# mbdriscoll/indigo

Measured on AMD Instinct MI355X. Metric: SENSE AHA evals/sec (256^3 x 8-coil non-Cartesian), higher is better.
Workload: dtype complex64 (f32)

## Files before the change

indigo_amd/csrc/ig_common.h:

```cpp
#pragma once

#include <hip/hip_runtime.h>
#include <cstdint>
#include <cstdio>
#include <cstdarg>
#include <string>
#include <type_traits>
#include <vector>

#include "indigo_hip.h"

struct ig_prof_rec {
    const char* name;
    double      bytes;
    hipEvent_t  e0, e1;
};

struct ig_ctx {
    int          device      = 0;
    hipStream_t  stream      = nullptr;
    bool         own_stream  = false;
    int          num_cu      = 256;
    std::string  err;
    double*      d_partials  = nullptr;
    double*      h_result    = nullptr;
    double*      d_scalars   = nullptr;
    void*        d_xpack     = nullptr;
    size_t       xpack_bytes = 0;
    void*        d_epg       = nullptr;
    size_t       epg_bytes   = 0;
    int32_t*     d_worklist  = nullptr;
    size_t       worklist_bytes = 0, partials_bytes = 0, scalars_bytes = 0;
    int          opt_fft_kernels = 0;
    int          opt_fft_zc = 1;
    bool         bricks_attr = false;
    bool         fft3d_attr = false;
    bool         fft_w32_attr = false;
    bool         fft_lds_attr = false;
    bool                     prof_on = false;
    bool                     capturing = false;
    std::vector<ig_prof_rec> prof;
    std::vector<hipEvent_t>  prof_pool;
};

struct ig_prof_scope {
    ig_ctx* ctx; size_t idx; bool on;
    ig_prof_scope(ig_ctx* c, const char* name, double bytes = 0.0) : ctx(c), idx(0), on(c && c->prof_on) {
        if (!on) return;
        ig_prof_rec r; r.name = name; r.bytes = bytes;
        auto get = [&]() { hipEvent_t e = nullptr;
            if (!ctx->prof_pool.empty()) { e = ctx->prof_pool.back(); ctx->prof_pool.pop_back(); }
            else (void)hipEventCreate(&e);
            return e; };
        r.e0 = get(); r.e1 = get();
        (void)hipEventRecord(r.e0, ctx->stream);
        idx = ctx->prof.size();
        ctx->prof.push_back(r);
    }
    ~ig_prof_scope() { if (on) (void)hipEventRecord(ctx->prof[idx].e1, ctx->stream); }
};

struct ig_graph {
    ig_ctx*        ctx  = nullptr;
    hipGraph_t     graph = nullptr;
    hipGraphExec_t exec = nullptr;
};

struct ig_event {
    ig_ctx*    ctx = nullptr;
    hipEvent_t ev  = nullptr;
};

constexpr int IG_MAX_RED_BLOCKS = 2048;
constexpr int IG_NUM_SCALARS = 1024;

std::string& ig_tls_error();

int ig_fail(ig_ctx* ctx, int code, const char* fmt, ...) __attribute__((format(printf, 3, 4)));

#define IG_HIP(ctx, call)                                                              \
    do {                                                                               \
        hipError_t e_ = (call);                                                        \
        if (e_ != hipSuccess)                                                          \
            return ig_fail((ctx), IG_ERR_HIP, "%s failed: %s (%s:%d)", #call,          \
                           hipGetErrorString(e_), __FILE__, __LINE__);                 \
    } while (0)

#define IG_REQUIRE(ctx, cond, ...)                                                     \
    do {                                                                               \
        if (!(cond)) return ig_fail((ctx), IG_ERR_ARG, __VA_ARGS__);                   \
    } while (0)

// ... 117 lines not shown
```

indigo_amd/csrc/ig_context.hip:

```cpp
#include "ig_common.h"
#include <cstring>

std::string& ig_tls_error() {
    static thread_local std::string e;
    return e;
}

int ig_fail(ig_ctx* ctx, int code, const char* fmt, ...) {
    char buf[1024];
    va_list ap;
    va_start(ap, fmt);
    vsnprintf(buf, sizeof(buf), fmt, ap);
    va_end(ap);
    ig_tls_error() = buf;
    if (ctx) ctx->err = buf;
    return code;
}

extern "C" {

int ig_abi_version(void) { return IG_ABI_VERSION; }

int ig_device_count(int* count) {
    if (!count) return ig_fail(nullptr, IG_ERR_ARG, "ig_device_count: count is NULL");
// ... 37 lines not shown
        ctx->own_stream = false;
    } else {
        if ((e = hipStreamCreateWithFlags(&ctx->stream, hipStreamNonBlocking)) != hipSuccess)
            return bail("hipStreamCreateWithFlags", e);
        ctx->own_stream = true;
    }
    ctx->partials_bytes = sizeof(double) * 2 * (IG_MAX_RED_BLOCKS + 1);
    if ((e = hipMalloc((void**)&ctx->d_partials, ctx->partials_bytes)) != hipSuccess)
        return bail("hipMalloc(partials)", e);
    if ((e = hipHostMalloc((void**)&ctx->h_result, sizeof(double) * 2, hipHostMallocDefault)) != hipSuccess)
        return bail("hipHostMalloc(result)", e);
    *out = ctx;
    return IG_OK;
}

int ig_init(int device_id, ig_ctx** out) { return ig_init_common(device_id, false, nullptr, out); }

int ig_init_on_stream(int device_id, void* hip_stream, ig_ctx** out) {
    return ig_init_common(device_id, true, hip_stream, out);
}

void ig_destroy(ig_ctx* ctx) {
    if (!ctx) return;
    (void)hipSetDevice(ctx->device);
    (void)hipStreamSynchronize(ctx->stream);
    for (ig_prof_rec& r : ctx->prof) { (void)hipEventDestroy(r.e0); (void)hipEventDestroy(r.e1); }
    for (hipEvent_t e : ctx->prof_pool) (void)hipEventDestroy(e);
    if (ctx->d_partials) (void)hipFree(ctx->d_partials);
    if (ctx->d_scalars) (void)hipFree(ctx->d_scalars);
    if (ctx->d_worklist) (void)hipFree(ctx->d_worklist);
    if (ctx->d_xpack) (void)hipFree(ctx->d_xpack);
    if (ctx->d_epg) (void)hipFree(ctx->d_epg);
    if (ctx->h_result) (void)hipHostFree(ctx->h_result);
    if (ctx->own_stream && ctx->stream) (void)hipStreamDestroy(ctx->stream);
    delete ctx;
}

const char* ig_last_error(ig_ctx* ctx) {
    if (ctx) return ctx->err.c_str();
    return ig_tls_error().c_str();
}

int ig_sync(ig_ctx* ctx) {
    IG_REQUIRE(ctx, ctx != nullptr, "ig_sync: ctx is NULL");
    if (int rc = ig_set_device(ctx)) return rc;
    IG_HIP(ctx, hipStreamSynchronize(ctx->stream));
    return IG_OK;
}

void* ig_stream(ig_ctx* ctx) { return ctx ? (void*)ctx->stream : nullptr; }

int ig_graph_begin(ig_ctx* ctx) {
    IG_REQUIRE(ctx, ctx != nullptr, "ig_graph_begin: ctx is NULL");
    IG_REQUIRE(ctx, !ctx->capturing, "ig_graph_begin: already recording");
    IG_REQUIRE(ctx, !ctx->prof_on, "ig_graph_begin: profile mode brackets launches with events of its own; switch it off");
    if (int rc = ig_set_device(ctx)) return rc;
    IG_HIP(ctx, hipStreamBeginCapture(ctx->stream, hipStreamCaptureModeThreadLocal));
    ctx->capturing = true;
    return IG_OK;
}

int ig_graph_end(ig_ctx* ctx, ig_graph** out) {
    IG_REQUIRE(ctx, ctx && out, "ig_graph_end: bad arguments");
    IG_REQUIRE(ctx, ctx->capturing, "ig_graph_end: not recording");
    *out = nullptr;
    ctx->capturing = false;
// ... 34 lines not shown
    ig_ctx* ctx = graph->ctx;
    IG_REQUIRE(ctx, !ctx->capturing, "ig_graph_launch: the context is recording");
    if (int rc = ig_set_device(ctx)) return rc;
    IG_HIP(ctx, hipGraphLaunch(graph->exec, ctx->stream));
    return IG_OK;
}

int ig_graph_destroy(ig_graph* graph) {
    if (!graph) return IG_OK;
    if (graph->exec) (void)hipGraphExecDestroy(graph->exec);
    if (graph->graph) (void)hipGraphDestroy(graph->graph);
    delete graph;
    return IG_OK;
}

int ig_device_name(ig_ctx* ctx, char* buf, size_t len) {
    IG_REQUIRE(ctx, ctx && buf && len > 0, "ig_device_name: bad arguments");
    hipDeviceProp_t prop;
    IG_HIP(ctx, hipGetDeviceProperties(&prop, ctx->device));
    snprintf(buf, len, "%s (%s, %d CUs)", prop.name, prop.gcnArchName, prop.multiProcessorCount);
    return IG_OK;
}

int ig_set_option(ig_ctx* ctx, const char* name, int64_t value) {
    IG_REQUIRE(ctx, ctx && name, "ig_set_option: bad arguments");
    if (std::string(name) == "fft.kernels") {
        IG_REQUIRE(ctx, value >= 0 && value <= 2, "ig_set_option: fft.kernels is 0 (all), 1 (no A x B passes) or 2 (generic stages only)");
        ctx->opt_fft_kernels = (int)value;
        return IG_OK;
    }
    if (std::string(name) == "fft.zc_intermediate") {
        IG_REQUIRE(ctx, value == 0 || value == 1, "ig_set_option: fft.zc_intermediate is 0 (the grid's order) or 1 (z-contiguous per kx tile)");
        ctx->opt_fft_zc = (int)value;
        return IG_OK;
    }
    return ig_fail(ctx, IG_ERR_ARG, "ig_set_option: unknown option '%s'", name);
}

int ig_library_bytes(ig_ctx* ctx, size_t* bytes) {
    IG_REQUIRE(ctx, ctx && bytes, "ig_library_bytes: bad arguments");
    *bytes = ctx->xpack_bytes + ctx->epg_bytes + (ctx->d_worklist ? ctx->worklist_bytes : 0) + (ctx->d_partials ? ctx->partials_bytes : 0) +
             (ctx->d_scalars ? ctx->scalars_bytes : 0);
    return IG_OK;
}

int ig_mem_info(ig_ctx* ctx, size_t* free_bytes, size_t* total_bytes) {
    IG_REQUIRE(ctx, ctx && free_bytes && total_bytes, "ig_mem_info: bad arguments");
    if (int rc = ig_set_device(ctx)) return rc;
    IG_HIP(ctx, hipMemGetInfo(free_bytes, total_bytes));
    return IG_OK;
}


int ig_malloc(ig_ctx* ctx, size_t nbytes, void** dptr) {
    IG_REQUIRE(ctx, ctx && dptr, "ig_malloc: bad arguments");
    if (int rc = ig_set_device(ctx)) return rc;
    *dptr = nullptr;
    size_t n = nbytes ? nbytes : 256;
    hipError_t e = hipMalloc(dptr, n);
    if (e == hipErrorOutOfMemory) {
        (void)hipGetLastError();
        return ig_fail(ctx, IG_ERR_NOMEM, "ig_malloc: out of device memory requesting %zu bytes", nbytes);
    }
    if (e != hipSuccess) return ig_fail(ctx, IG_ERR_HIP, "hipMalloc(%zu) failed: %s", nbytes, hipGetErrorString(e));
    return IG_OK;
}
// ... 156 lines not shown
```

indigo_amd/csrc/ig_fft.hip:

```cpp
#include "ig_common.h"
#include "ig_packed.h"
#include "ig_fft_ab.h"
#include "ig_fft_plan.h"
#include "ig_fft_regs.h"

namespace {


template <int R1, int R2, int T, int W, bool AXIS0, int WMODE, bool BOXED, int HALF>
__global__ void __launch_bounds__(W * T, (!AXIS0 && R1 == 32 && (W == 32 || HALF == 1 || HALF == 3)) ? 4 : 1)
k_fft_2stage(PassDesc d, const float2* __restrict__ tw) {
    constexpr int n = R1 * R2, B1 = R2 / T, B2 = R1 / T, NT = W * T;
    constexpr bool NT_LD = true, NT_ST = true;
    constexpr bool HALF_IN = HALF == 1 || HALF == 3, HALF_OUT = HALF == 2 || HALF == 4;
    constexpr int SUMW = WMODE >= 3 ? (1 << (WMODE - 3)) : 0;
    constexpr bool SINV = HALF_OUT;
    const bool inv = (HALF_OUT || HALF_IN) ? false : (d.inverse != 0);
    static_assert(R2 % T == 0 && R1 % T == 0 && T == 16 && B1 == 1, "lane groups of 16, one stage-1 butterfly per thread");
    extern __shared__ float2 lds[];
    float2* __restrict__ tws = lds + (AXIS0 ? 16 * 17 * W : 16 * T * W);
    const int tid = threadIdx.x;
    constexpr int TWN = n / NT;
    constexpr bool TW_LATE = (n % NT == 0) && TWN <= 2;
    float2 tw_mine[TW_LATE ? TWN : 1];
    if (TW_LATE) {
#pragma unroll
        for (int i = 0; i < TWN; ++i) tw_mine[i] = tw[n + tid + i * NT];
    } else for (int k = tid; k < n; k += NT) tws[k] = tw[n + k];

    const int t = AXIS0 ? (tid % T) : (tid / W);
    const int w = AXIS0 ? (tid / T) : (tid % W);
    unsigned tr, k1, k2;
    pass_tile(d, tr, k1, k2);
    const int64_t k0u = (int64_t)tr * ((!AXIS0 && d.cw) ? (d.cw_log2 >= 0 ? W >> d.cw_log2 : W / d.cw) : W);
    int in_lo = d.in_lo, in_hi = d.in_hi, out_lo = d.out_lo, out_hi = d.out_hi;
    short2 k1r = make_short2(0, 0x7fff), trg = make_short2(0, 0x7fff);
    PassRecords rcd{0u, 0u, 0x7fff0000u, 0xffffffffu, false, false, false, true, false};
    if (BOXED && !AXIS0) rcd = pass_records(d, tw, tr, k1, 16, t, true);
    const bool has_k1r = rcd.has_k1r, has_trg = rcd.has_trg, has_zb = rcd.has_zb;
    int64_t o_in = k0u * d.in_s[0], o_out = k0u * d.out_s[0];
    if (BOXED && !AXIS0 && WMODE == 0 && d.zc_log2) {
        const int64_t q = k0u >> d.zc_log2, e = k0u - (q << d.zc_log2);
        if (d.in_zt) o_in = q * d.in_zt + e;
        if (d.out_zt) o_out = q * d.out_zt + e;
    }
    const float2* const b_in = d.in + (o_in + (int64_t)k1 * d.in_s[1] + (int64_t)k2 * d.in_s[2]);
// ... 194 lines not shown
               "ig_fft: axis stride too large for the %s kernel", kernel);
    return IG_OK;
}

bool ig_two_stage_variant(const AxisPlan& ax, const PassDesc& d, bool axis0, int wmode, bool& boxed, int& half) {
    boxed = d.tile_range || !(d.in_lo <= 0 && d.in_hi >= (int)ax.n && d.out_lo <= 0 && d.out_hi >= (int)ax.n);
    const int qn = (int)ax.n / 4;
    half = 0;
    if (boxed) {
        const bool in_full = d.in_lo <= 0 && d.in_hi >= (int)ax.n, out_full = d.out_lo <= 0 && d.out_hi >= (int)ax.n;
        if (d.in_lo == qn && d.in_hi == 3 * qn && !(d.tile_range && d.tile_range_mode == 2))
            half = (out_full && !d.tile_range && !d.tile_bits) ? 3 : 1;
        else if (d.out_lo == qn && d.out_hi == 3 * qn && !(d.tile_range && d.tile_range_mode == 1))
            half = (in_full && !d.tile_range && !d.tile_bits) ? 4 : 2;
        if (wmode == 1 && half != 3) half = 0;
        if (wmode >= 2 && half != 4) half = 0;
        if (((half == 1 || half == 3) && d.inverse) || ((half == 2 || half == 4) && !d.inverse)) half = 0;
    }
    const bool big_stride = (d.in_sj > d.out_sj ? d.in_sj : d.out_sj) * 8 >= (1 << 20);
    const bool w32_generic = half == 0 && (big_stride || d.tile_bits != nullptr);
    const bool w32 = (ax.n == 512 && !axis0 && wmode == 0 && !d.cw && d.ext0 % 32 == 0 &&
        (half == 1 || half == 3 || half == 2 || half == 4 || w32_generic) &&
        (!d.tile_range || d.tile_shift >= 1));
    return d.wide ? d.wide == 2 : w32;
}


typedef void (*Kernel2S)(PassDesc, const float2*);
template <int WM, int HF> struct V2 {};
template <typename... P> struct V2List {};
using V2_BOXED = V2List<V2<0, 0>, V2<0, 1>, V2<0, 2>, V2<0, 3>, V2<0, 4>, V2<1, 0>, V2<1, 3>, V2<2, 0>, V2<2, 4>>;
using V2_SUM = V2List<V2<3, 0>, V2<3, 4>, V2<4, 0>, V2<4, 4>, V2<5, 0>, V2<5, 4>, V2<6, 0>, V2<6, 4>, V2<7, 0>, V2<7, 4>>;
using V2_W32 = V2List<V2<0, 0>, V2<0, 1>, V2<0, 2>, V2<0, 3>, V2<0, 4>>;
template <int R1, int W, bool AXIS0, int... WM, int... HF>
static Kernel2S pick_2stage(V2List<V2<WM, HF>...>, int wm, int half) {
    Kernel2S k = nullptr;
    ((wm == WM && half == HF ? (void)(k = &k_fft_2stage<R1, 16, 16, W, AXIS0, WM, true, HF>) : (void)0), ...);
    return k;
}

int ig_launch_2stage(ig_ctx* ctx, const AxisPlan& ax, const PassDesc& d_in, bool axis0, int wmode) {
    PassDesc d = d_in;
    if (d.ncols == 0) return IG_OK;
    IG_REQUIRE(ctx, !d.tile_bits || d.tile_words == 16 || d.tile_words == 0, "ig_fft: the two-stage kernel reads support bitmaps of 16 words per entry (got %d)", d.tile_words);
    const int64_t cpt = (!axis0 && d.cw) ? ax.W / d.cw : ax.W;
    IG_REQUIRE(ctx, !d.cw || (!axis0 && d.cw <= ax.W && ax.W % d.cw == 0), "ig_fft: bad lane split");
    dim3 grid, block((unsigned)(ax.W * ax.T));
    if (int rc = ig_pass_tiles(ctx, d, cpt, axis0 ? ax.n + 15 : 3 * (ax.n / 16) + 15, wmode != 0, "two-stage", grid)) return rc;
    size_t lds = ax.lds_bytes;
    bool boxed; int half;
    Kernel2S k = nullptr;
    if (ig_two_stage_variant(ax, d, axis0, wmode, boxed, half)) {
        if (d.tile_range) d.tile_shift -= 1;
        grid = pass_grid(d, d.ext0 / 32); block = dim3(512);
        lds = ((size_t)16 * 16 * 32 + 512) * 8;
        if (!ctx->fft_w32_attr) {
            for (int h = 0; h <= 4; ++h)
                IG_HIP(ctx, hipFuncSetAttribute(reinterpret_cast<const void*>(pick_2stage<32, 32, false>(V2_W32{}, 0, h)), hipFuncAttributeMaxDynamicSharedMemorySize, (int)lds));
            ctx->fft_w32_attr = true;
        }
        k = pick_2stage<32, 32, false>(V2_W32{}, 0, half);
    } else {
        IG_REQUIRE(ctx, wmode != 3 || (!axis0 && d.cw >= 1), "ig_fft: the coil-summing pass is a strided pass with a lane split");
        const int wm = wmode == 3 ? 3 + d.cw_log2 : wmode;
        with_flag(ax.n == 512, [&](auto n512) { with_flag(axis0, [&](auto a0) {
            constexpr int R1 = decltype(n512)::value ? 32 : 16;
            constexpr bool A0 = decltype(a0)::value;
            if (!boxed && wm == 0) k = &k_fft_2stage<R1, 16, 16, 16, A0, 0, false, 0>;
            else if (wm < 3) k = pick_2stage<R1, 16, A0>(V2_BOXED{}, wm, half);
            else if constexpr (!A0) k = pick_2stage<R1, 16, false>(V2_SUM{}, wm, half);
        }); });
    }
    IG_REQUIRE(ctx, k, "ig_fft: no two-stage kernel for weight mode %d", wmode);
    hipLaunchKernelGGL(k, grid, block, lds, ctx->stream, d, ax.d_tw);
    IG_LAUNCH_CHECK(ctx, "k_fft_2stage");
    return IG_OK;
}
```

indigo_amd/csrc/ig_fft_plan.h:

```cpp
#pragma once
#include "ig_common.h"
#include "ig_fft_ab.h"
#include <memory>
#include <string>
#include <vector>

namespace {

constexpr int MAX_STAGES = 16;
constexpr int E = 8;
constexpr int LDS_NMAX = 4096;
constexpr size_t LDS_BUDGET = 150 * 1024;

struct Radices { int r[MAX_STAGES]; };

}

struct Chirp;
struct AxisPlan {
    int64_t n = 1, inner = 1, outer = 1;
    int kind = 2;
    std::shared_ptr<Chirp> chirp;
    int nstages = 0;
    int ab_A = 0, ab_B = 0;
// ... 14 lines not shown
    float2* d_in_s[2] = {nullptr, nullptr};
    float2* d_hat_out_s[2] = {nullptr, nullptr};
    AxisPlan sub;
    bool fused = false;
    ~Chirp() {
        for (int d = 0; d < 2; ++d) { if (d_b[d]) (void)hipFree(d_b[d]); if (d_bhat[d]) (void)hipFree(d_bhat[d]); if (d_bout[d]) (void)hipFree(d_bout[d]);
                                      if (d_hat_out[d]) (void)hipFree(d_hat_out[d]);
                                      if (d_in_s[d]) (void)hipFree(d_in_s[d]); if (d_hat_out_s[d]) (void)hipFree(d_hat_out_s[d]); }
        if (sub.d_tw) (void)hipFree(sub.d_tw);
    }
};

struct ig_fft {
    ig_ctx* ctx = nullptr;
    bool is_chirp_sub = false;
    int rank = 0;
    int64_t dims[3] = {1, 1, 1};
    int64_t batch = 1;
    int64_t total = 0;
    AxisPlan axis[3];
    size_t workspace_bytes = 0;
    std::string desc;
    bool two_launch = false;
    size_t inplace_workspace_bytes = 0;
    bool padded = false;
    bool has_ab_axis = false;
    bool has_chirp_axis = false;
    int zw_in = 16, zw_out = 16;
    int layout = 0;
    int support_tile = 16;
    int64_t box_lo[3] = {0, 0, 0}, box_dims[3] = {1, 1, 1};
};

int ig_launch_2stage(ig_ctx* ctx, const AxisPlan& ax, const PassDesc& d, bool axis0, int wmode);
bool ig_two_stage_variant(const AxisPlan& ax, const PassDesc& d, bool axis0, int wmode, bool& boxed, int& half);
int ig_pass_tiles(ig_ctx* ctx, PassDesc& d, int64_t cpt, int64_t reach, bool weights, const char* kernel, dim3& grid);

int ig_launch_fft3d_a(ig_ctx* ctx, const float2* in, float2* out, const float2* tw, int64_t batch, int inverse);
int ig_launch_fft3d_b(ig_ctx* ctx, const float2* in, float2* out, const float2* tw, int64_t batch, int inverse);
int ig_launch_fft_lds(ig_ctx* ctx, const AxisPlan& ax, const float2* in, float2* out, int inverse);
int ig_launch_fft_generic_stage(ig_ctx* ctx, unsigned blocks, const float2* in, float2* out, const float2* tw, int64_t n, int64_t inner,
                                int64_t total, int R, int64_t Ns, int inverse);
int ig_launch_chirp_pre(ig_ctx* ctx, unsigned blocks, const float2* x, float2* W, const float2* b, int64_t n, int64_t m, int64_t inner, int64_t total_m);
int ig_launch_chirp_mul(ig_ctx* ctx, unsigned blocks, float2* W, const float2* bhat, int64_t m, int64_t inner, int64_t total_m);
int ig_launch_chirp_post(ig_ctx* ctx, unsigned blocks, const float2* W, float2* y, const float2* bout, int64_t n, int64_t m, int64_t inner, int64_t total_n);
```

indigo_amd/csrc/ig_fft_plan.hip:

```cpp
#include "ig_common.h"
#include "ig_fft_ab.h"
#include "ig_fft_ab_list.h"
#include "ig_fft_zc.h"
#include "ig_fft_plan.h"
#include <algorithm>
#include <array>
#include <cmath>
#include <complex>
#include <functional>

namespace {

bool factor_lds(int64_t n, Radices& rad, int& nstages) {
    nstages = 0;
    int64_t m = n;
    auto push = [&](int r) { rad.r[nstages++] = r; };
    while (m % 8 == 0 && nstages < MAX_STAGES) { push(8); m /= 8; }
    while (m % 4 == 0 && nstages < MAX_STAGES) { push(4); m /= 4; }
    while (m % 2 == 0 && nstages < MAX_STAGES) { push(2); m /= 2; }
    for (int p : {3, 5, 7})
        while (m % p == 0 && nstages < MAX_STAGES) { push(p); m /= p; }
    return m == 1;
}

void factor_generic(int64_t n, std::vector<int64_t>& out) {
    out.clear();
    int64_t m = n;
    while (m % 8 == 0) { out.push_back(8); m /= 8; }
    while (m % 4 == 0) { out.push_back(4); m /= 4; }
    while (m % 2 == 0) { out.push_back(2); m /= 2; }
    for (int64_t p = 3; p * p <= m; p += 2)
        while (m % p == 0) { out.push_back(p); m /= p; }
    if (m > 1) out.push_back(m);
}

int64_t largest_prime_factor(int64_t n) {
// ... 266 lines not shown
        }
        upload(hat_out_s[dir], 2 * (size_t)m);
    }
    if (err != hipSuccess) {
        for (int d = 0; d < 2; ++d) { if (in_s[d]) (void)hipFree(in_s[d]); if (hat_out_s[d]) (void)hipFree(hat_out_s[d]); }
        return ig_fail(ctx, IG_ERR_HIP, "ig_fft_set_axis_shift: the tables of a shift by %lld points could not be uploaded: %s", (long long)c, hipGetErrorString(err));
    }
    for (int d = 0; d < 2; ++d) { ch.d_in_s[d] = in_s[d]; ch.d_hat_out_s[d] = hat_out_s[d]; }
    ch.shift = c;
    return IG_OK;
}

int launch_chirp_desc(ig_ctx* ctx, const AxisPlan& ax, const PassDesc& d_in) {
    const Chirp& ch = *ax.chirp;
    IG_REQUIRE(ctx, ch.fused, "ig_fft: this chirp-z axis has no one-launch route");
    IG_REQUIRE(ctx, !d_in.cw && (!d_in.tile_bits || d_in.tile_words == ch.sub.ab_B), "ig_fft: a chirp-z pass takes no lane split, and support bitmaps of B = %d words per entry", ch.sub.ab_B);
    IG_REQUIRE(ctx, d_in.in_lo >= 0 && d_in.in_hi <= ax.n && d_in.out_lo >= 0 && d_in.out_hi <= ax.n, "ig_fft: chirp-z boxes must lie inside the axis");
    PassDesc d = d_in;
    if (d.ncols == 0) return IG_OK;
    const int dir = d.inverse ? 1 : 0;
    d.w = ch.d_b[dir]; d.w2 = ch.d_hat_out[dir]; d.chirp_out = 0;
    if (ch.shift) { d.w = ch.d_in_s[dir]; d.w2 = ch.d_hat_out_s[dir]; d.chirp_out = 1; }
    dim3 grid;
    if (int rc = ig_pass_tiles(ctx, d, anyfft::AB_W, ch.sub.ab_B - 1, false, "chirp-z", grid)) return rc;
    const dim3 block((unsigned)(anyfft::AB_W * ch.sub.ab_B));
    const int r = launch_part(ABZ_PARTS, ctx->stream, ch.m, grid, block, d, ch.sub.d_tw);
    if (r == 2) return ig_fail(ctx, IG_ERR_UNSUPPORTED, "ig_fft: device %d refused the LDS the chirp-z kernel over %lld points needs", ctx->device, (long long)ch.m);
    if (!r)
        return ig_fail(ctx, IG_ERR_UNSUPPORTED, "ig_fft: no chirp-z kernel for m = %lld", (long long)ch.m);
    IG_LAUNCH_CHECK(ctx, "k_fft_chirp");
    return IG_OK;
}

int launch_pass(ig_ctx* ctx, const AxisPlan& ax, const PassDesc& d, bool axis0, int wmode) {
    if (ax.kind == 3) return ig_launch_2stage(ctx, ax, d, axis0, wmode);
    if (ax.kind == 5) {
        IG_REQUIRE(ctx, !axis0 && wmode == 0, "ig_fft: a chirp-z axis takes unweighted strided passes only");
        return launch_chirp_desc(ctx, ax, d);
    }
    IG_REQUIRE(ctx, ax.kind == 4 && !axis0, "ig_fft: a zero-padded pass on an axis without a two-stage kernel");
    return launch_ab_desc(ctx, ax, d, wmode);
}

}

extern "C" {

int ig_fft_plan(ig_ctx* ctx, int rank, const int64_t* dims, int64_t batch, ig_fft** plan, size_t* workspace_bytes) {
    IG_REQUIRE(ctx, ctx && dims && plan, "ig_fft_plan: bad arguments");
    IG_REQUIRE(ctx, rank >= 1 && rank <= 3, "ig_fft_plan: rank %d not in 1..3", rank);
    IG_REQUIRE(ctx, batch >= 1, "ig_fft_plan: batch must be >= 1");
    *plan = nullptr;
    if (int rc = ig_set_device(ctx)) return rc;
    ig_fft* p = new ig_fft();
    p->ctx = ctx; p->rank = rank; p->batch = batch;
    p->total = batch;
    for (int a = 0; a < rank; ++a) {
        if (dims[a] < 1) { delete p; return ig_fail(ctx, IG_ERR_ARG, "ig_fft_plan: dims[%d] = %lld", a, (long long)dims[a]); }
        p->dims[a] = dims[a];
        p->total *= dims[a];
    }
    bool need_ws = false;
    for (int a = 0; a < rank; ++a) {
        int rc = plan_axis(ctx, p, a);
        if (rc != IG_OK) { ig_fft_destroy(p); return rc; }
        if (p->axis[a].kind == 1) need_ws = true;
    }
    p->workspace_bytes = need_ws ? (size_t)p->total * 8 : 0;
// ... 288 lines not shown
    if (g.snt) {
        d.tile_range = support; d.tile_range_mode = inverse ? 2 : 1; d.tile_range_k1 = g.snt; d.tile_shift = g.tile_shift;
    }
    if (support) {
        d.tile_bits = reinterpret_cast<const uint32_t*>(support + g.bits) + (inverse ? 0 : g.bits_out);
        d.tile_words = inverse ? g.zw_in : g.zw_out;
        if (inverse) d.k1_range = support + g.hull_y;
    }
    return d;
}

static bool zc_route(const ig_fft* p, const PaddedGeom& g, float2* zc, bool inverse, int64_t z0, PassDesc& dy, PassDesc& dz) {
    if (!p->ctx->opt_fft_zc || !g.interleaved || !zc || p->axis[1].kind != 3 || p->axis[2].kind != 3) return false;
    bool by, bz; int half;
    const bool wy = ig_two_stage_variant(p->axis[1], dy, false, 0, by, half), wz = ig_two_stage_variant(p->axis[2], dz, false, 0, bz, half);
    if (!by || !bz || (wy && !wz)) return false;
    const ZcGeom z{g.n[0], g.n[1], g.b[2], g.C, wz ? 32 : 16};
    if (!zc_valid(z)) return false;
    const ZcSide sy = zc_side(z, 1), sz = zc_side(z, 2);
    float2* const y_base = zc + zc_offset(z, 0, 0, z0, 0);
    float2* const z_base = zc - g.l[2] * sz.sj;
    if (!inverse) {
        dy.out = y_base; dy.out_sj = sy.sj; dy.out_s[0] = 1; dy.out_s[1] = sy.s1; dy.out_s[2] = 0; dy.out_zt = sy.zt;
        dz.in = z_base;  dz.in_sj = sz.sj;  dz.in_s[0] = 1;  dz.in_s[1] = sz.s1;  dz.in_s[2] = 0;  dz.in_zt = sz.zt;
    } else {
        dz.out = z_base; dz.out_sj = sz.sj; dz.out_s[0] = 1; dz.out_s[1] = sz.s1; dz.out_s[2] = 0; dz.out_zt = sz.zt;
        dy.in = y_base;  dy.in_sj = sy.sj;  dy.in_s[0] = 1;  dy.in_s[1] = sy.s1;  dy.in_s[2] = 0;  dy.in_zt = sy.zt;
    }
    dy.zc_log2 = dz.zc_log2 = sz.piece_log2;
    dy.wide = wy ? 2 : 1; dz.wide = wz ? 2 : 1;
    return true;
}

static int exec_padded(ig_fft* p, float2* x, int64_t x_bstride, const float2* w, float2* y, float2* work, const short2* support) {
    ig_ctx* ctx = p->ctx;
    const PaddedGeom g = padded_geom(p, false, x_bstride, false);
    const PaddedBufs m = padded_bufs(p, g, x, y, y, work);
    const int64_t plane = g.n[0] * g.n[1], b2 = g.b[2];
    PassDesc dy = pass_y(g, false, m, support, 0, b2), dz = pass_z(g, false, m, support);
    zc_route(p, g, work, false, 0, dy, dz);
    {
        ig_prof_scope prof(ctx, "fft_pad_x", (double)(g.bvol + (w ? g.bvol : 0) + g.cvol) * g.C * 8.0);
        int wmode; bool axis0;
        const PassDesc d = pass_x(g, false, m, w, 0, b2, false, wmode, axis0);
        if (int rc = launch_pass(ctx, p->axis[0], d, axis0, wmode)) return rc;
    }
    {
        ig_prof_scope prof(ctx, "fft_pad_y", (double)(g.cvol + plane * b2) * g.C * 8.0);
        if (int rc = launch_pass(ctx, p->axis[1], dy, false, 0)) return rc;
    }
    {
        ig_prof_scope prof(ctx, "fft_pad_z", (double)(plane * b2 + g.vol) * g.C * 8.0);
        if (int rc = launch_pass(ctx, p->axis[2], dz, false, 0)) return rc;
    }
    return IG_OK;
}

static int exec_cropped(ig_fft* p, float2* y, const float2* w, float2* x, int64_t x_bstride, float2* work, const short2* support,
                        bool sum_coils, int phases, int64_t z0, int64_t z1) {
    ig_ctx* ctx = p->ctx;
    const PaddedGeom g = padded_geom(p, true, x_bstride, sum_coils);
    const PaddedBufs m = padded_bufs(p, g, x, y, work, work);
    const int64_t plane = g.n[0] * g.n[1], b2 = g.b[2];
    const int64_t nz = z1 - z0;
    PassDesc dy = pass_y(g, true, m, support, z0, nz > 0 ? nz : 0), dz = pass_z(g, true, m, support);
    zc_route(p, g, work, true, z0, dy, dz);
    if (phases & 1) {
        ig_prof_scope prof(ctx, "fft_crop_z", (double)(g.vol + plane * b2) * g.C * 8.0);
        if (int rc = launch_pass(ctx, p->axis[2], dz, false, 0)) return rc;
    }
    if (!(phases & 2) || nz <= 0) return IG_OK;
    {
        ig_prof_scope prof(ctx, "fft_crop_y", (double)(plane * nz + g.n[0] * g.b[1] * nz) * g.C * 8.0);
        if (int rc = launch_pass(ctx, p->axis[1], dy, false, 0)) return rc;
    }
    {
        const double bytes = sum_coils ? (double)(g.cvol + g.bvol) * g.C * 8.0 + (double)g.bvol * 8.0 : (double)(g.cvol + g.bvol + (w ? g.bvol : 0)) * g.C * 8.0;
        ig_prof_scope prof(ctx, "fft_crop_x", bytes * (double)nz / (double)b2);
        int wmode; bool axis0;
        const PassDesc d = pass_x(g, true, m, w, z0, nz, sum_coils, wmode, axis0);
        if (int rc = launch_pass(ctx, p->axis[0], d, axis0, wmode)) return rc;
    }
    return IG_OK;
}

int64_t ig_fft_zc_size(const int64_t* dims, const int64_t* box_dims, int64_t coils, int64_t piece_bytes) {
    if (!dims || !box_dims || piece_bytes < 8 || piece_bytes % 8) return -1;
    const ZcGeom z{dims[0], dims[1], box_dims[2], coils, piece_bytes / 8};
    return zc_valid(z) && box_dims[2] <= dims[2] ? zc_size(z) * 8 : -1;
}

int64_t ig_fft_zc_offset(const int64_t* dims, const int64_t* box_dims, int64_t coils, int64_t piece_bytes, int64_t kx, int64_t ky, int64_t z, int64_t coil) {
    if (ig_fft_zc_size(dims, box_dims, coils, piece_bytes) < 0) return -1;
    const ZcGeom g{dims[0], dims[1], box_dims[2], coils, piece_bytes / 8};
    if (kx < 0 || kx >= g.n0 || ky < 0 || ky >= g.n1 || z < 0 || z >= g.b2 || coil < 0 || coil >= g.C) return -1;
    return zc_offset(g, kx, ky, z, coil) * 8;
}

int ig_fft_support_words(int64_t n, int* zw_in, int* zw_out) {
    if (!zw_in || !zw_out) return ig_fail(nullptr, IG_ERR_ARG, "ig_fft_support_words: bad arguments");
    int A = 0, B = 0;
    if (n == 256 || n == 512) { *zw_in = *zw_out = 16; return IG_OK; }
    if (abd_supported(n) && ab_split(n, A, B)) { *zw_in = B; *zw_out = A; return IG_OK; }
    {
        const int64_t big = largest_prime_factor(n);
        if (big > 7 && n >= 32 && chirp_ab_length(n, A, B) && n <= 32 * (int64_t)B) { *zw_in = *zw_out = B; return IG_OK; }
    }
    return ig_fail(nullptr, IG_ERR_UNSUPPORTED, "ig_fft_support_words: no zero-pad-aware z pass for an axis of %lld points", (long long)n);
}

int ig_fft_padded_axis_kind(int64_t n, int* kind) {
    if (!kind || n < 1) return ig_fail(nullptr, IG_ERR_ARG, "ig_fft_padded_axis_kind: bad arguments");
    int A = 0, B = 0;
    *kind = 0;
    if (n == 256 || n == 512) { *kind = 3; return IG_OK; }
    if (abd_supported(n)) { *kind = 4; return IG_OK; }
// ... 105 lines not shown
```

Baseline: 169.0.

## Chunk x/y FFT passes by z-planes across streams with cache-retaining stores

Splits the padded and cropped FFT x/y pass pair into z-plane chunks of about 128 MiB each, runs them round-robin across up to three streams joined by events, and gives the first pass of each pair ordinary (temporal) stores so the second pass can find its input in cache. The aim is to cut the round trip to HBM between the x and y passes and to overlap chunks on separate streams. This adds more kernel launches, stream fork/join overhead, and new kernel template instantiations, and it is turned off during graph capture.

```diff
diff --git a/indigo_amd/csrc/ig_common.h b/indigo_amd/csrc/ig_common.h
--- a/indigo_amd/csrc/ig_common.h
+++ b/indigo_amd/csrc/ig_common.h
@@ -33,6 +33,9 @@
     size_t       worklist_bytes = 0, partials_bytes = 0, scalars_bytes = 0;
     int          opt_fft_kernels = 0;
     int          opt_fft_zc = 1;
+    int          opt_fft_xy_planes = -1, opt_fft_xy_streams = 2;
+    hipStream_t  xy_stream[2] = {nullptr, nullptr};
+    hipEvent_t   xy_fork = nullptr, xy_join[2] = {nullptr, nullptr};
     bool         bricks_attr = false;
     bool         fft3d_attr = false;
     bool         fft_w32_attr = false;
@@ -44,8 +47,8 @@
 };
 
 struct ig_prof_scope {
-    ig_ctx* ctx; size_t idx; bool on;
-    ig_prof_scope(ig_ctx* c, const char* name, double bytes = 0.0) : ctx(c), idx(0), on(c && c->prof_on) {
+    ig_ctx* ctx; size_t idx; bool on; hipStream_t stream;
+    ig_prof_scope(ig_ctx* c, const char* name, double bytes = 0.0, hipStream_t s = nullptr) : ctx(c), idx(0), on(c && c->prof_on), stream(s ? s : c ? c->stream : nullptr) {
         if (!on) return;
         ig_prof_rec r; r.name = name; r.bytes = bytes;
         auto get = [&]() { hipEvent_t e = nullptr;
@@ -53,11 +56,11 @@
             else (void)hipEventCreate(&e);
             return e; };
         r.e0 = get(); r.e1 = get();
-        (void)hipEventRecord(r.e0, ctx->stream);
+        (void)hipEventRecord(r.e0, stream);
         idx = ctx->prof.size();
         ctx->prof.push_back(r);
     }
-    ~ig_prof_scope() { if (on) (void)hipEventRecord(ctx->prof[idx].e1, ctx->stream); }
+    ~ig_prof_scope() { if (on) (void)hipEventRecord(ctx->prof[idx].e1, stream); }
 };
 
 struct ig_graph {
diff --git a/indigo_amd/csrc/ig_context.hip b/indigo_amd/csrc/ig_context.hip
--- a/indigo_amd/csrc/ig_context.hip
+++ b/indigo_amd/csrc/ig_context.hip
@@ -93,6 +93,11 @@
     if (ctx->d_xpack) (void)hipFree(ctx->d_xpack);
     if (ctx->d_epg) (void)hipFree(ctx->d_epg);
     if (ctx->h_result) (void)hipHostFree(ctx->h_result);
+    for (int i = 0; i < 2; ++i) {
+        if (ctx->xy_stream[i]) (void)hipStreamDestroy(ctx->xy_stream[i]);
+        if (ctx->xy_join[i]) (void)hipEventDestroy(ctx->xy_join[i]);
+    }
+    if (ctx->xy_fork) (void)hipEventDestroy(ctx->xy_fork);
     if (ctx->own_stream && ctx->stream) (void)hipStreamDestroy(ctx->stream);
     delete ctx;
 }
@@ -193,6 +198,16 @@
     if (std::string(name) == "fft.zc_intermediate") {
         IG_REQUIRE(ctx, value == 0 || value == 1, "ig_set_option: fft.zc_intermediate is 0 (the grid's order) or 1 (z-contiguous per kx tile)");
         ctx->opt_fft_zc = (int)value;
+        return IG_OK;
+    }
+    if (std::string(name) == "fft.xy_chunk_planes") {
+        IG_REQUIRE(ctx, value >= -1 && value <= 0x7fffffffLL, "ig_set_option: fft.xy_chunk_planes is 0 (one launch per pass), the image planes per chunk of the x / y pair, or -1 (chunks of 128 MiB)");
+        ctx->opt_fft_xy_planes = (int)value;
+        return IG_OK;
+    }
+    if (std::string(name) == "fft.xy_chunk_streams") {
+        IG_REQUIRE(ctx, value >= 1 && value <= 3, "ig_set_option: fft.xy_chunk_streams is 1, 2 or 3 (the context's stream and up to two more)");
+        ctx->opt_fft_xy_streams = (int)value;
         return IG_OK;
     }
     return ig_fail(ctx, IG_ERR_ARG, "ig_set_option: unknown option '%s'", name);
diff --git a/indigo_amd/csrc/ig_fft.hip b/indigo_amd/csrc/ig_fft.hip
--- a/indigo_amd/csrc/ig_fft.hip
+++ b/indigo_amd/csrc/ig_fft.hip
@@ -7,11 +7,11 @@
 namespace {
 
 
-template <int R1, int R2, int T, int W, bool AXIS0, int WMODE, bool BOXED, int HALF>
+template <int R1, int R2, int T, int W, bool AXIS0, int WMODE, bool BOXED, int HALF, bool KEEP_ST = false>
 __global__ void __launch_bounds__(W * T, (!AXIS0 && R1 == 32 && (W == 32 || HALF == 1 || HALF == 3)) ? 4 : 1)
 k_fft_2stage(PassDesc d, const float2* __restrict__ tw) {
     constexpr int n = R1 * R2, B1 = R2 / T, B2 = R1 / T, NT = W * T;
-    constexpr bool NT_LD = true, NT_ST = true;
+    constexpr bool NT_LD = true, NT_ST = !KEEP_ST;
     constexpr bool HALF_IN = HALF == 1 || HALF == 3, HALF_OUT = HALF == 2 || HALF == 4;
     constexpr int SUMW = WMODE >= 3 ? (1 << (WMODE - 3)) : 0;
     constexpr bool SINV = HALF_OUT;
@@ -272,14 +272,16 @@
 using V2_BOXED = V2List<V2<0, 0>, V2<0, 1>, V2<0, 2>, V2<0, 3>, V2<0, 4>, V2<1, 0>, V2<1, 3>, V2<2, 0>, V2<2, 4>>;
 using V2_SUM = V2List<V2<3, 0>, V2<3, 4>, V2<4, 0>, V2<4, 4>, V2<5, 0>, V2<5, 4>, V2<6, 0>, V2<6, 4>, V2<7, 0>, V2<7, 4>>;
 using V2_W32 = V2List<V2<0, 0>, V2<0, 1>, V2<0, 2>, V2<0, 3>, V2<0, 4>>;
-template <int R1, int W, bool AXIS0, int... WM, int... HF>
+using V2_KEEP = V2List<V2<0, 0>, V2<0, 2>, V2<0, 4>, V2<1, 0>, V2<1, 3>>;
+using V2_W32_KEEP = V2List<V2<0, 0>, V2<0, 2>, V2<0, 4>>;
+template <int R1, int W, bool AXIS0, bool KEEP = false, int... WM, int... HF>
 static Kernel2S pick_2stage(V2List<V2<WM, HF>...>, int wm, int half) {
     Kernel2S k = nullptr;
-    ((wm == WM && half == HF ? (void)(k = &k_fft_2stage<R1, 16, 16, W, AXIS0, WM, true, HF>) : (void)0), ...);
+    ((wm == WM && half == HF ? (void)(k = &k_fft_2stage<R1, 16, 16, W, AXIS0, WM, true, HF, KEEP>) : (void)0), ...);
     return k;
 }
 
-int ig_launch_2stage(ig_ctx* ctx, const AxisPlan& ax, const PassDesc& d_in, bool axis0, int wmode) {
+int ig_launch_2stage(ig_ctx* ctx, const AxisPlan& ax, const PassDesc& d_in, bool axis0, int wmode, hipStream_t stream, bool keep_out) {
     PassDesc d = d_in;
     if (d.ncols == 0) return IG_OK;
     IG_REQUIRE(ctx, !d.tile_bits || d.tile_words == 16 || d.tile_words == 0, "ig_fft: the two-stage kernel reads support bitmaps of 16 words per entry (got %d)", d.tile_words);
@@ -295,11 +297,15 @@
         grid = pass_grid(d, d.ext0 / 32); block = dim3(512);
         lds = ((size_t)16 * 16 * 32 + 512) * 8;
         if (!ctx->fft_w32_attr) {
-            for (int h = 0; h <= 4; ++h)
+            for (int h = 0; h <= 4; ++h) {
                 IG_HIP(ctx, hipFuncSetAttribute(reinterpret_cast<const void*>(pick_2stage<32, 32, false>(V2_W32{}, 0, h)), hipFuncAttributeMaxDynamicSharedMemorySize, (int)lds));
+                if (Kernel2S kk = pick_2stage<32, 32, false, true>(V2_W32_KEEP{}, 0, h))
+                    IG_HIP(ctx, hipFuncSetAttribute(reinterpret_cast<const void*>(kk), hipFuncAttributeMaxDynamicSharedMemorySize, (int)lds));
+            }
             ctx->fft_w32_attr = true;
         }
-        k = pick_2stage<32, 32, false>(V2_W32{}, 0, half);
+        if (keep_out) k = pick_2stage<32, 32, false, true>(V2_W32_KEEP{}, 0, half);
+        if (!k) k = pick_2stage<32, 32, false>(V2_W32{}, 0, half);
     } else {
         IG_REQUIRE(ctx, wmode != 3 || (!axis0 && d.cw >= 1), "ig_fft: the coil-summing pass is a strided pass with a lane split");
         const int wm = wmode == 3 ? 3 + d.cw_log2 : wmode;
@@ -307,12 +313,15 @@
             constexpr int R1 = decltype(n512)::value ? 32 : 16;
             constexpr bool A0 = decltype(a0)::value;
             if (!boxed && wm == 0) k = &k_fft_2stage<R1, 16, 16, 16, A0, 0, false, 0>;
-            else if (wm < 3) k = pick_2stage<R1, 16, A0>(V2_BOXED{}, wm, half);
+            else if (wm < 3) {
+                if constexpr (!A0) { if (keep_out) k = pick_2stage<R1, 16, false, true>(V2_KEEP{}, wm, half); }
+                if (!k) k = pick_2stage<R1, 16, A0>(V2_BOXED{}, wm, half);
+            }
             else if constexpr (!A0) k = pick_2stage<R1, 16, false>(V2_SUM{}, wm, half);
         }); });
     }
     IG_REQUIRE(ctx, k, "ig_fft: no two-stage kernel for weight mode %d", wmode);
-    hipLaunchKernelGGL(k, grid, block, lds, ctx->stream, d, ax.d_tw);
+    hipLaunchKernelGGL(k, grid, block, lds, stream ? stream : ctx->stream, d, ax.d_tw);
     IG_LAUNCH_CHECK(ctx, "k_fft_2stage");
     return IG_OK;
 }
diff --git a/indigo_amd/csrc/ig_fft_plan.h b/indigo_amd/csrc/ig_fft_plan.h
--- a/indigo_amd/csrc/ig_fft_plan.h
+++ b/indigo_amd/csrc/ig_fft_plan.h
@@ -70,7 +70,7 @@
     int64_t box_lo[3] = {0, 0, 0}, box_dims[3] = {1, 1, 1};
 };
 
-int ig_launch_2stage(ig_ctx* ctx, const AxisPlan& ax, const PassDesc& d, bool axis0, int wmode);
+int ig_launch_2stage(ig_ctx* ctx, const AxisPlan& ax, const PassDesc& d, bool axis0, int wmode, hipStream_t stream = nullptr, bool keep_out = false);
 bool ig_two_stage_variant(const AxisPlan& ax, const PassDesc& d, bool axis0, int wmode, bool& boxed, int& half);
 int ig_pass_tiles(ig_ctx* ctx, PassDesc& d, int64_t cpt, int64_t reach, bool weights, const char* kernel, dim3& grid);
 
diff --git a/indigo_amd/csrc/ig_fft_plan.hip b/indigo_amd/csrc/ig_fft_plan.hip
--- a/indigo_amd/csrc/ig_fft_plan.hip
+++ b/indigo_amd/csrc/ig_fft_plan.hip
@@ -2,6 +2,7 @@
 #include "ig_fft_ab.h"
 #include "ig_fft_ab_list.h"
 #include "ig_fft_zc.h"
+#include "ig_fft_xy.h"
 #include "ig_fft_plan.h"
 #include <algorithm>
 #include <array>
@@ -334,8 +335,9 @@
     return IG_OK;
 }
 
-int launch_pass(ig_ctx* ctx, const AxisPlan& ax, const PassDesc& d, bool axis0, int wmode) {
-    if (ax.kind == 3) return ig_launch_2stage(ctx, ax, d, axis0, wmode);
+int launch_pass(ig_ctx* ctx, const AxisPlan& ax, const PassDesc& d, bool axis0, int wmode, hipStream_t stream = nullptr, bool keep_out = false) {
+    if (ax.kind == 3) return ig_launch_2stage(ctx, ax, d, axis0, wmode, stream, keep_out);
+    IG_REQUIRE(ctx, !stream && !keep_out, "ig_fft: only two-stage passes run on a stream of their own");
     if (ax.kind == 5) {
         IG_REQUIRE(ctx, !axis0 && wmode == 0, "ig_fft: a chirp-z axis takes unweighted strided passes only");
         return launch_chirp_desc(ctx, ax, d);
@@ -690,6 +692,35 @@
     return true;
 }
 
+static XyChunks xy_partition(const ig_fft* p, const PaddedGeom& g, int64_t z0, int64_t z1) {
+    const ig_ctx* ctx = p->ctx;
+    const bool chunked = ctx->opt_fft_xy_planes != 0 && g.interleaved && p->axis[0].kind == 3 && p->axis[1].kind == 3 && !ctx->capturing;
+    const int64_t K = ctx->opt_fft_xy_planes < 0 ? xy_auto_planes(g.n[0] * g.b[1] * g.C * 8) : ctx->opt_fft_xy_planes;
+    return xy_chunks(z0, z1, chunked ? K : 0, chunked ? ctx->opt_fft_xy_streams : 1);
+}
+
+static hipStream_t xy_stream(ig_ctx* ctx, int i) { return i == 0 ? nullptr : ctx->xy_stream[i - 1]; }
+
+static int xy_fork(ig_ctx* ctx, const XyChunks& part) {
+    if (part.S <= 1) return IG_OK;
+    if (!ctx->xy_fork) IG_HIP(ctx, hipEventCreateWithFlags(&ctx->xy_fork, hipEventDisableTiming));
+    IG_HIP(ctx, hipEventRecord(ctx->xy_fork, ctx->stream));
+    for (int i = 0; i < part.S - 1; ++i) {
+        if (!ctx->xy_stream[i]) IG_HIP(ctx, hipStreamCreateWithFlags(&ctx->xy_stream[i], hipStreamNonBlocking));
+        if (!ctx->xy_join[i]) IG_HIP(ctx, hipEventCreateWithFlags(&ctx->xy_join[i], hipEventDisableTiming));
+        IG_HIP(ctx, hipStreamWaitEvent(ctx->xy_stream[i], ctx->xy_fork, 0));
+    }
+    return IG_OK;
+}
+
+static int xy_join(ig_ctx* ctx, const XyChunks& part) {
+    for (int i = 0; i < part.S - 1; ++i) {
+        IG_HIP(ctx, hipEventRecord(ctx->xy_join[i], ctx->xy_stream[i]));
+        IG_HIP(ctx, hipStreamWaitEvent(ctx->stream, ctx->xy_join[i], 0));
+    }
+    return IG_OK;
+}
+
 static int exec_padded(ig_fft* p, float2* x, int64_t x_bstride, const float2* w, float2* y, float2* work, const short2* support) {
     ig_ctx* ctx = p->ctx;
     const PaddedGeom g = padded_geom(p, false, x_bstride, false);
@@ -697,21 +728,34 @@
     const int64_t plane = g.n[0] * g.n[1], b2 = g.b[2];
     PassDesc dy = pass_y(g, false, m, support, 0, b2), dz = pass_z(g, false, m, support);
     zc_route(p, g, work, false, 0, dy, dz);
-    {
-        ig_prof_scope prof(ctx, "fft_pad_x", (double)(g.bvol + (w ? g.bvol : 0) + g.cvol) * g.C * 8.0);
-        int wmode; bool axis0;
-        const PassDesc d = pass_x(g, false, m, w, 0, b2, false, wmode, axis0);
-        if (int rc = launch_pass(ctx, p->axis[0], d, axis0, wmode)) return rc;
-    }
-    {
-        ig_prof_scope prof(ctx, "fft_pad_y", (double)(g.cvol + plane * b2) * g.C * 8.0);
-        if (int rc = launch_pass(ctx, p->axis[1], dy, false, 0)) return rc;
-    }
-    {
-        ig_prof_scope prof(ctx, "fft_pad_z", (double)(plane * b2 + g.vol) * g.C * 8.0);
-        if (int rc = launch_pass(ctx, p->axis[2], dz, false, 0)) return rc;
-    }
-    return IG_OK;
+    const XyChunks part = xy_partition(p, g, 0, b2);
+    if (int rc = xy_fork(ctx, part)) return rc;
+    const bool keep = part.count > 1;
+    int rc = IG_OK;
+    for (int64_t i = 0; i < part.count && !rc; ++i) {
+        const XyChunk c = xy_chunk(part, i);
+        hipStream_t const s = xy_stream(ctx, c.stream);
+        const double share = (double)c.nz / (double)b2;
+        {
+            ig_prof_scope prof(ctx, "fft_pad_x", (double)(g.bvol + (w ? g.bvol : 0) + g.cvol) * g.C * 8.0 * share, s);
+            int wmode; bool axis0;
+            const PassDesc d = pass_x(g, false, m, w, c.z0, c.nz, false, wmode, axis0);
+            rc = launch_pass(ctx, p->axis[0], d, axis0, wmode, s, keep);
+        }
+        if (rc) break;
+        PassDesc dyc = dy;
+        if (part.count > 1) {
+            PassDesc dzc = pass_z(g, false, m, support);
+            dyc = pass_y(g, false, m, support, c.z0, c.nz);
+            zc_route(p, g, work, false, c.z0, dyc, dzc);
+        }
+        ig_prof_scope prof(ctx, "fft_pad_y", (double)(g.cvol + plane * b2) * g.C * 8.0 * share, s);
+        rc = launch_pass(ctx, p->axis[1], dyc, false, 0, s);
+    }
+    if (int rj = xy_join(ctx, part)) return rc ? rc : rj;
+    if (rc) return rc;
+    ig_prof_scope prof(ctx, "fft_pad_z", (double)(plane * b2 + g.vol) * g.C * 8.0);
+    return launch_pass(ctx, p->axis[2], dz, false, 0);
 }
 
 static int exec_cropped(ig_fft* p, float2* y, const float2* w, float2* x, int64_t x_bstride, float2* work, const short2* support,
@@ -728,18 +772,32 @@
         if (int rc = launch_pass(ctx, p->axis[2], dz, false, 0)) return rc;
     }
     if (!(phases & 2) || nz <= 0) return IG_OK;
-    {
-        ig_prof_scope prof(ctx, "fft_crop_y", (double)(plane * nz + g.n[0] * g.b[1] * nz) * g.C * 8.0);
-        if (int rc = launch_pass(ctx, p->axis[1], dy, false, 0)) return rc;
-    }
-    {
-        const double bytes = sum_coils ? (double)(g.cvol + g.bvol) * g.C * 8.0 + (double)g.bvol * 8.0 : (double)(g.cvol + g.bvol + (w ? g.bvol : 0)) * g.C * 8.0;
-        ig_prof_scope prof(ctx, "fft_crop_x", bytes * (double)nz / (double)b2);
+    const double bytes_x = sum_coils ? (double)(g.cvol + g.bvol) * g.C * 8.0 + (double)g.bvol * 8.0 : (double)(g.cvol + g.bvol + (w ? g.bvol : 0)) * g.C * 8.0;
+    const XyChunks part = xy_partition(p, g, z0, z1);
+    if (int rc = xy_fork(ctx, part)) return rc;
+    const bool keep = part.count > 1;
+    int rc = IG_OK;
+    for (int64_t i = 0; i < part.count && !rc; ++i) {
+        const XyChunk c = xy_chunk(part, i);
+        hipStream_t const s = xy_stream(ctx, c.stream);
+        {
+            PassDesc dyc = dy;
+            if (part.count > 1) {
+                PassDesc dzc = pass_z(g, true, m, support);
+                dyc = pass_y(g, true, m, support, c.z0, c.nz);
+                zc_route(p, g, work, true, c.z0, dyc, dzc);
+            }
+            ig_prof_scope prof(ctx, "fft_crop_y", (double)(plane * c.nz + g.n[0] * g.b[1] * c.nz) * g.C * 8.0, s);
+            rc = launch_pass(ctx, p->axis[1], dyc, false, 0, s, keep);
+        }
+        if (rc) break;
+        ig_prof_scope prof(ctx, "fft_crop_x", bytes_x * (double)c.nz / (double)b2, s);
         int wmode; bool axis0;
-        const PassDesc d = pass_x(g, true, m, w, z0, nz, sum_coils, wmode, axis0);
-        if (int rc = launch_pass(ctx, p->axis[0], d, axis0, wmode)) return rc;
-    }
-    return IG_OK;
+        const PassDesc d = pass_x(g, true, m, w, c.z0, c.nz, sum_coils, wmode, axis0);
+        rc = launch_pass(ctx, p->axis[0], d, axis0, wmode, s);
+    }
+    if (int rj = xy_join(ctx, part)) return rc ? rc : rj;
+    return rc;
 }
 
 int64_t ig_fft_zc_size(const int64_t* dims, const int64_t* box_dims, int64_t coils, int64_t piece_bytes) {
diff --git a/indigo_amd/csrc/ig_fft_xy.h b/indigo_amd/csrc/ig_fft_xy.h
--- /dev/null
+++ b/indigo_amd/csrc/ig_fft_xy.h
@@ -0,0 +1,34 @@
+#pragma once
+#include <cstdint>
+
+constexpr int XY_MAX_STREAMS = 3;
+
+struct XyChunks {
+    int64_t z0, z1;
+    int64_t K;
+    int64_t count;
+    int S;
+};
+
+struct XyChunk { int64_t z0, nz; int stream; };
+
+constexpr int64_t XY_AUTO_CHUNK_BYTES = int64_t(128) << 20;
+static inline int64_t xy_auto_planes(int64_t plane_bytes) {
+    return plane_bytes <= 0 ? 0 : (XY_AUTO_CHUNK_BYTES + plane_bytes - 1) / plane_bytes;
+}
+
+static inline XyChunks xy_chunks(int64_t z0, int64_t z1, int64_t K, int S) {
+    XyChunks p{z0, z1, 0, 0, 1};
+    const int64_t planes = z1 - z0;
+    if (planes <= 0) return p;
+    p.K = (K <= 0 || K >= planes) ? planes : K;
+    p.count = (planes + p.K - 1) / p.K;
+    p.S = S < 1 ? 1 : S > XY_MAX_STREAMS ? XY_MAX_STREAMS : S;
+    if (p.S > p.count) p.S = (int)p.count;
+    return p;
+}
+
+static inline XyChunk xy_chunk(const XyChunks& p, int64_t i) {
+    const int64_t lo = p.z0 + i * p.K, hi = lo + p.K < p.z1 ? lo + p.K : p.z1;
+    return XyChunk{lo, hi - lo, (int)(i % p.S)};
+}
```

Measured after the change: 177.3 (median of 6 runs). 4.9% higher.
